# g1mv/density

Hardware: NVIDIA H100
Metric: chameleon_encode_input_GBps (higher is better)
Workload: dtype u32

## Files before the change

### density_b200/csrc/chameleon_encode.cu

```cuda
#include <cstdio>
#include "common.cuh"
#include "encode_internal.cuh"

namespace dns {
namespace cham {

constexpr int TILE_Q = 4096;
__device__ __forceinline__ bool bit_test(const uint32_t* bm, uint32_t i) { return (bm[i >> 5] >> (i & 31)) & 1u; }

constexpr int F6_THREADS = 512, F6_QPT = 8;
constexpr int F6_NW = F6_THREADS / 32, F6_WQ = 32 * F6_QPT;
static_assert(F6_THREADS * F6_QPT == TILE_Q, "tile geometry");
constexpr int F6_MB_SLOTS = 4096, F6_MB_CAP = 4;
constexpr int F6_SEC_SLOTS = 64, F6_SEC_CAP = 16;
#ifdef DNS_PHASE_TIMING
__device__ long long g_f6_ph[8];
#define F6_PH(k) { if (threadIdx.x == 0 && blockIdx.x == 77) { long long tn = clock64(); g_f6_ph[k] += tn - f6_tprev; f6_tprev = tn; } }
#define F6_PH_DECL long long f6_tprev = clock64();
#else
#define F6_PH(k)
#define F6_PH_DECL
#endif
constexpr uint32_t F6_TOUCHED = 1u << 12, F6_DROPPED = 1u << 13;
struct Flag6Smem {
    uint16_t tab[65536];
    uint32_t vbit[2048];
    uint2 rec[TILE_Q];
    union {
        uint16_t mb[F6_MB_SLOTS][F6_MB_CAP];
        uint2 stage[F6_NW][64];
    };
    uint32_t mbcnt[2][F6_MB_SLOTS / 4];
    __align__(16) uint32_t sec[F6_SEC_SLOTS][F6_SEC_CAP];
    uint32_t seccnt[2][F6_SEC_SLOTS];
    uint32_t sigw[2][TILE_Q / 32];
    uint32_t cnt[32];
    uint32_t unres_count;
    uint32_t overflow;
};
static_assert(sizeof(Flag6Smem) <= 227 * 1024, "flag pass shared memory");

__device__ __forceinline__ void f6_append_unres(bool pred, uint32_t qidx_in_run, uint32_t hf, uint32_t* s_count, uint2* __restrict__ unres_run) {
    const uint32_t m = __ballot_sync(0xFFFFFFFFu, pred);
    if (m == 0) return;
    uint32_t base = 0;
    if ((threadIdx.x & 31) == 0) base = atomicAdd(s_count, (uint32_t)__popc(m));
    base = __shfl_sync(0xFFFFFFFFu, base, 0);
    if (pred) {
        const uint32_t idx = base + __popc(m & lanemask_lt());
        if (idx < 65536u) unres_run[idx] = make_uint2(qidx_in_run, hf);
    }
}

static_assert(F6_NW == 16, "one warp per bucket class hash >> 12");
__device__ __forceinline__ void f6_replay_step(Flag6Smem& S, const uint2* stage, uint32_t n, uint32_t buf, uint32_t run_q0,
                                               uint2* __restrict__ unres_run) {
    const uint32_t lane = threadIdx.x & 31;
    const bool valid = lane < n;
    uint2 r = make_uint2(0, 0);
    if (valid) r = stage[lane];
    const uint32_t hh = r.x & 0xFFFFu, ff = r.x >> 16, pos = r.y & 0xFFFu;
    uint32_t cur = 0;
    if (valid) cur = S.tab[hh];
    const uint32_t grp = __match_any_sync(0xFFFFFFFFu, valid ? hh : 0x10000u + lane);
    const uint32_t lower = grp & lanemask_lt();
    const uint32_t fprev = __shfl_sync(0xFFFFFFFFu, ff, lower ? 31 - __clz(lower) : 0);
    bool touched = true, hit;
    if (lower) hit = fprev == ff;
    else {
        if (cur == 0) touched = bit_test(S.vbit, hh);
        hit = touched && cur == ff;
    }
    if (valid && (grp & lanemask_gt()) == 0) {
        S.tab[hh] = (uint16_t)ff;
        if (ff == 0) atomicOr(&S.vbit[hh >> 5], 1u << (hh & 31));
    }
    if (valid && hit) atomicOr(&S.sigw[buf][pos >> 5], 1u << (pos & 31));
    f6_append_unres(valid && !touched, run_q0 + pos, r.x, &S.unres_count, unres_run);
    __syncwarp();
}

__device__ __noinline__ void f6_replay(Flag6Smem& S, uint32_t buf, uint32_t run_q0, uint2* __restrict__ unres_run) {
    const uint32_t lane = threadIdx.x & 31, warp = threadIdx.x >> 5;
    {
        const uint32_t n = S.cnt[warp];
        const uint2* __restrict__ myrec = S.rec + warp * F6_WQ;
        #pragma unroll 1
        for (uint32_t i = lane; i < n; i += 32) {
            const uint2 r = myrec[i];
            S.tab[r.x & 0xFFFFu] = (uint16_t)(r.y >> 16);
        }
    }
    __syncthreads();
    uint2* __restrict__ stage = S.stage[warp];
    uint32_t ns = 0;
    #pragma unroll 1
    for (uint32_t w = 0; w < (uint32_t)F6_NW; ++w) {
        const uint32_t n = S.cnt[w];
        const uint2* __restrict__ rg = S.rec + w * F6_WQ;
        #pragma unroll 1
        for (uint32_t i0 = 0; i0 < n; i0 += 32) {
            const uint32_t i = i0 + lane;
            uint2 r = make_uint2(0, 0);
            if (i < n) r = rg[i];
            const bool mine = i < n && ((r.x & 0xFFFFu) >> 12) == warp;
            const uint32_t m = __ballot_sync(0xFFFFFFFFu, mine);
            if (mine) stage[ns + __popc(m & lanemask_lt())] = r;
            ns += __popc(m);
            if (ns >= 32) {
                __syncwarp();
                f6_replay_step(S, stage, 32, buf, run_q0, unres_run);
                const uint2 rest = stage[32 + lane];
                __syncwarp();
                if (lane < ns - 32) stage[lane] = rest;
                ns -= 32;
                __syncwarp();
            }
        }
    }
    __syncwarp();
    if (ns) f6_replay_step(S, stage, ns, buf, run_q0, unres_run);
}

template <bool GENERIC>
__device__ __forceinline__ void f6_tile(Flag6Smem& S, const uint32_t (&q)[F6_QPT], uint32_t validmask, uint32_t buf, uint32_t run_q0,
                                        uint2* __restrict__ unres_run) {
    const uint32_t tid = threadIdx.x, lane = tid & 31, warp = tid >> 5;
    const uint32_t pos0 = warp * F6_WQ + lane;
    uint32_t h[F6_QPT], f[F6_QPT], old[F6_QPT];
    uint32_t missmask = 0;
    F6_PH_DECL
#pragma unroll
    for (int k = 0; k < F6_MB_SLOTS / 4 / F6_THREADS; ++k) S.mbcnt[buf ^ 1u][tid + k * F6_THREADS] = 0;
    if (tid < F6_SEC_SLOTS) S.seccnt[buf ^ 1u][tid] = 0;
#pragma unroll
    for (int j = 0; j < F6_QPT; ++j) {
        const uint32_t p = hash_prod(q[j]);
        h[j] = prod_hash(p);
        f[j] = prod_fp(p, q[j]);
        old[j] = S.tab[h[j]];
    }
    uint32_t fmin = f[0];
#pragma unroll
    for (int j = 0; j < F6_QPT; ++j) {
        bool miss = old[j] != f[j];
        if (GENERIC) miss = miss && ((validmask >> j) & 1u);
        if (miss) missmask |= 1u << j;
        fmin = min(fmin, f[j]);
    }
    if (fmin == 0) {
#pragma unroll
        for (int j = 0; j < F6_QPT; ++j)
            if (f[j] == 0 && old[j] == 0 && (!GENERIC || ((validmask >> j) & 1u)) && !bit_test(S.vbit, h[j])) missmask |= 1u << j;
    }
    __syncthreads();
    F6_PH(0)
#pragma unroll
    for (int j = 0; j < F6_QPT; ++j)
        if (missmask & (1u << j)) S.tab[h[j]] = (uint16_t)f[j];
    __syncthreads();
    F6_PH(1)
    uint32_t clean[F6_QPT], base = 0;
    uint2* __restrict__ myrec = S.rec + warp * F6_WQ;
#pragma unroll
    for (int j = 0; j < F6_QPT; ++j) {
        bool dirty = (missmask >> j) & 1u;
        if (!dirty) dirty = S.tab[h[j]] != f[j];
        if (GENERIC) dirty = dirty && ((validmask >> j) & 1u);
        const uint32_t db = __ballot_sync(0xFFFFFFFFu, dirty);
        clean[j] = GENERIC ? __ballot_sync(0xFFFFFFFFu, !dirty && ((validmask >> j) & 1u)) : ~db;
        if (dirty) myrec[base + __popc(db & lanemask_lt())] = make_uint2(h[j] | (f[j] << 16), (pos0 + 32 * j) | (old[j] << 16));
        base += __popc(db);
    }
    if (lane == 0) {
#pragma unroll
        for (int j = 0; j < F6_QPT; j += 4)
            *reinterpret_cast<uint4*>(&S.sigw[buf][warp * F6_QPT + j]) = make_uint4(clean[j], clean[j + 1], clean[j + 2], clean[j + 3]);
        S.cnt[warp] = base;
    }
    __syncwarp();
    uint2 r0 = make_uint2(0, 0);
    bool drop0 = false;
    {
        uint32_t carry_x = 0, carry_pos = 0;
        #pragma unroll 1
        for (uint32_t i0 = 0; i0 < base; i0 += 32) {
            const uint32_t i = i0 + lane;
            const bool valid = i < base;
            uint2 r = make_uint2(0xFFFFFFFFu, 0);
            if (valid) {
                r = myrec[i];
                if ((r.y >> 16) != 0 || bit_test(S.vbit, r.x & 0xFFFFu)) r.y |= F6_TOUCHED;
            }
            uint32_t px = __shfl_up_sync(0xFFFFFFFFu, r.x, 1), ppos = __shfl_up_sync(0xFFFFFFFFu, r.y & 0xFFFu, 1);
            if (lane == 0) { px = carry_x; ppos = carry_pos; }
            const bool drop = valid && i != 0 && px == r.x && ppos + 1 == (r.y & 0xFFFu);
            carry_x = __shfl_sync(0xFFFFFFFFu, r.x, 31); carry_pos = __shfl_sync(0xFFFFFFFFu, r.y & 0xFFFu, 31);
            if (i0 == 0) { r0 = r; drop0 = drop; }
            if (drop) {
                const uint32_t pos = r.y & 0xFFFu;
                atomicOr(&S.sigw[buf][pos >> 5], 1u << (pos & 31));
                if (i0) myrec[i].y = r.y | F6_DROPPED;
            } else if (valid) {
                if (i0 && (r.y & F6_TOUCHED)) myrec[i].y = r.y;
                const uint32_t hh = r.x & 0xFFFFu, slot = hh & (F6_MB_SLOTS - 1), sh = (slot & 3u) * 8u;
                const uint32_t k = (atomicAdd(&S.mbcnt[buf][slot >> 2], 1u << sh) >> sh) & 0xFFu;
                if (k < (uint32_t)F6_MB_CAP) S.mb[slot][k] = (uint16_t)(((hh >> 12) << 12) | (warp * F6_WQ + i));
                else {
                    const uint32_t s2 = slot & (F6_SEC_SLOTS - 1);
                    const uint32_t k2 = atomicAdd(&S.seccnt[buf][s2], 1u);
                    if (k2 < (uint32_t)F6_SEC_CAP) S.sec[s2][k2] = (hh << 12) | (warp * F6_WQ + i);
                    else S.overflow = 1;
                }
            }
        }
    }
    __syncthreads();
    F6_PH(2)
#ifdef DNS_PHASE_TIMING
    if (threadIdx.x == 0 && blockIdx.x == 77) { g_f6_ph[6] += S.overflow; uint32_t tot = 0; for (int w = 0; w < F6_NW; ++w) tot += S.cnt[w]; g_f6_ph[7] += tot; }
#endif
    if (S.overflow) {
        f6_replay(S, buf, run_q0, unres_run);
    } else {
        #pragma unroll 1
        for (uint32_t i0 = 0; i0 < base; i0 += 32) {
            const uint32_t i = i0 + lane;
            bool valid = i < base;
            uint2 r = r0;
            if (i0) r = valid ? myrec[i] : make_uint2(0, 0);
            if (i0 ? (r.y & F6_DROPPED) != 0 : drop0) valid = false;
            const uint32_t hh = r.x & 0xFFFFu, ff = r.x >> 16, pos = r.y & 0xFFFu, slot = hh & (F6_MB_SLOTS - 1);
            const uint32_t myidx = warp * F6_WQ + i;
            bool later = false, hit = false, unres = false;
            if (valid) {
                const uint32_t n = (S.mbcnt[buf][slot >> 2] >> ((slot & 3u) * 8u)) & 0xFFu;
                const uint2 e2 = *reinterpret_cast<const uint2*>(&S.mb[slot][0]);
                const uint32_t me = ((hh >> 12) << 12) | myidx;
                int best = -1;
#pragma unroll
                for (int t = 0; t < F6_MB_CAP; ++t) {
                    const uint32_t e = ((t & 2) ? e2.y : e2.x) >> ((t & 1) * 16) & 0xFFFFu;
                    if ((uint32_t)t < n && ((e ^ me) >> 12) == 0) {
                        if (e < me) best = max(best, (int)(e & 0xFFFu));
                        later |= e > me;
                    }
                }
                if (n > (uint32_t)F6_MB_CAP) {
                    const uint32_t s2 = slot & (F6_SEC_SLOTS - 1);
                    const uint32_t n2 = S.seccnt[buf][s2];
                    const uint32_t mine = (hh << 12) | myidx;
                    #pragma unroll 1
                    for (uint32_t t4 = 0; t4 < n2; t4 += 4) {
                        const uint4 e4 = *reinterpret_cast<const uint4*>(&S.sec[s2][t4]);
                        const uint32_t ev[4] = {e4.x, e4.y, e4.z, e4.w};
#pragma unroll
                        for (int t = 0; t < 4; ++t) {
                            const uint32_t e = ev[t];
                            if (t4 + t < n2 && ((e ^ mine) & 0xFFFFF000u) == 0) {
                                if (e < mine) best = max(best, (int)(e & 0xFFFu));
                                later |= e > mine;
                            }
                        }
                    }
                }
                if (best >= 0) hit = (S.rec[best].x >> 16) == ff;
                else if (r.y & F6_TOUCHED) hit = (r.y >> 16) == ff;
                else unres = true;
                if (!later) {
                    S.tab[hh] = (uint16_t)ff;
                    if (ff == 0) atomicOr(&S.vbit[hh >> 5], 1u << (hh & 31));
                }
                if (hit) atomicOr(&S.sigw[buf][pos >> 5], 1u << (pos & 31));
            }
            f6_append_unres(unres, run_q0 + pos, r.x, &S.unres_count, unres_run);
        }
    }
    __syncthreads();
    F6_PH(3)
}

__global__ void __launch_bounds__(F6_THREADS, 1)
cham_flag_pass6(const uint32_t* __restrict__ in, uint64_t nquads, uint32_t tiles_total, uint32_t nruns,
                uint32_t* __restrict__ sigw_g, uint2* __restrict__ unres, uint32_t* __restrict__ unres_count,
                uint32_t* __restrict__ final_tab, const uint8_t* __restrict__ copymap, const Status* __restrict__ gate)
{
    if (gate && !(gate->nonquiet && !gate->converged)) return;
    extern __shared__ __align__(16) unsigned char smem_raw[];
    Flag6Smem& S = *reinterpret_cast<Flag6Smem*>(smem_raw);
    const uint32_t tid = threadIdx.x, lane = tid & 31, warp = tid >> 5;
    const uint32_t run = blockIdx.x;
    const uint64_t t_begin = (uint64_t)run * tiles_total / nruns;
    const uint64_t t_end = (uint64_t)(run + 1) * tiles_total / nruns;
    uint2* __restrict__ unres_run = unres + (size_t)run * 65536;
    const uint32_t pos0 = warp * F6_WQ + lane;
    const uint32_t ntile_run = (uint32_t)(t_end - t_begin);
    const uint64_t q_begin = t_begin * TILE_Q;
    const uint64_t q_end64 = (t_end * TILE_Q < nquads) ? t_end * TILE_Q : nquads;
    const uint32_t run_quads = q_begin < q_end64 ? (uint32_t)(q_end64 - q_begin) : 0u;
    const uint32_t* __restrict__ rin = in + q_begin;
    uint32_t* __restrict__ rsig = sigw_g + t_begin * (TILE_Q / 32);
    const uint8_t* __restrict__ rcm = copymap ? copymap + t_begin * 64 : nullptr;
    {
        const uint4 z = make_uint4(0, 0, 0, 0);
        uint4* t4 = reinterpret_cast<uint4*>(S.tab);
        #pragma unroll 1
        for (uint32_t i = tid; i < 65536 * 2 / 16; i += F6_THREADS) t4[i] = z;
        #pragma unroll 1
        for (uint32_t i = tid; i < 2048; i += F6_THREADS) S.vbit[i] = 0;
        #pragma unroll 1
        for (uint32_t i = tid; i < F6_MB_SLOTS / 4; i += F6_THREADS) { S.mbcnt[0][i] = 0; S.mbcnt[1][i] = 0; }
        if (tid < F6_SEC_SLOTS) { S.seccnt[0][tid] = 0; S.seccnt[1][tid] = 0; }
        if (tid == 0) { S.unres_count = 0; S.overflow = 0; }
    }
    __syncthreads();
    uint32_t nxt[F6_QPT], nxt2[F6_QPT];
#pragma unroll
    for (int j = 0; j < F6_QPT; ++j) {
        nxt[j] = (pos0 + 32 * j < run_quads) ? ld_stream_u32(rin + pos0 + 32 * j) : 0u;
        nxt2[j] = (TILE_Q + pos0 + 32 * j < run_quads) ? ld_stream_u32(rin + TILE_Q + pos0 + 32 * j) : 0u;
    }
    #pragma unroll 1
    for (uint32_t lt = 0; lt < ntile_run; ++lt) {
        uint32_t q[F6_QPT];
        const uint32_t run_q0 = lt * TILE_Q;
        const uint32_t left = run_q0 < run_quads ? run_quads - run_q0 : 0u;
        const uint32_t buf = lt & 1u;
#pragma unroll
        for (int j = 0; j < F6_QPT; ++j) { q[j] = nxt[j]; nxt[j] = nxt2[j]; }
        {
            const uint32_t nleft = left > 2u * TILE_Q ? left - 2u * TILE_Q : 0u;
            const uint32_t* __restrict__ np = rin + run_q0 + 2 * TILE_Q + pos0;
            if (nleft >= (uint32_t)TILE_Q) {
#pragma unroll
                for (int j = 0; j < F6_QPT; ++j) nxt2[j] = ld_stream_u32(np + 32 * j);
            } else {
#pragma unroll
                for (int j = 0; j < F6_QPT; ++j) nxt2[j] = (pos0 + 32 * j < nleft) ? ld_stream_u32(np + 32 * j) : 0u;
            }
        }
        if (left >= (uint32_t)TILE_Q && !rcm) {
            f6_tile<false>(S, q, (1u << F6_QPT) - 1u, buf, run_q0, unres_run);
        } else {
            uint32_t validmask = 0, cp = 0;
            if (rcm) {
#pragma unroll
                for (int b = 0; b < F6_WQ / 64; ++b) cp |= (rcm[lt * 64 + warp * (F6_WQ / 64) + b] ? 1u : 0u) << b;
            }
#pragma unroll
            for (int j = 0; j < F6_QPT; ++j)
                if (pos0 + 32 * j < left && !((cp >> (j >> 1)) & 1u)) validmask |= 1u << j;
            f6_tile<true>(S, q, validmask, buf, run_q0, unres_run);
        }
        if (tid < TILE_Q / 32) rsig[lt * (TILE_Q / 32) + tid] = S.sigw[buf][tid];
        if (tid == 0) S.overflow = 0;
    }
    #pragma unroll 1
    for (uint32_t i = tid; i < 65536; i += F6_THREADS) {
        const uint32_t v = S.tab[i];
        const uint32_t tch = (v != 0 || bit_test(S.vbit, i)) ? 0x10000u : 0u;
        final_tab[(size_t)run * 65536 + i] = v | tch;
    }
    if (tid == 0) unres_count[run] = S.unres_count < 65536u ? S.unres_count : 65536u;
#ifdef DNS_PHASE_TIMING
    if (tid == 0 && run == 77 && ntile_run) { const long long nt = ntile_run;
        printf("f6 run %u tiles %lld cycles/tile: A %lld B %lld C+deposit %lld D+S4 %lld  overflow tiles %lld dirty/tile %lld\n", run, nt, g_f6_ph[0] / nt, g_f6_ph[1] / nt,
               g_f6_ph[2] / nt, g_f6_ph[3] / nt, g_f6_ph[6], g_f6_ph[7] / nt);
        for (int k = 0; k < 8; ++k) g_f6_ph[k] = 0; }
#endif
}

__device__ __forceinline__ bool gate_open(const Status* g) { return !g || (g->nonquiet && !g->converged); }

__global__ void cham_carry_scan(const uint32_t* __restrict__ final_tab, const uint32_t* __restrict__ init, int init_untouched,
                                uint32_t nruns, uint32_t* __restrict__ carry, uint32_t* __restrict__ table_out,
                                const Status* __restrict__ gate = nullptr) {
    if (!gate_open(gate)) return;
    uint32_t hb = blockIdx.x * blockDim.x + threadIdx.x;
    if (hb >= 65536) return;
    uint32_t c = init ? init[hb] : ((hb == 0 && !init_untouched) ? 0x10000u : 0u);
    for (uint32_t r = 0; r < nruns; ++r) {
        if (carry) carry[(size_t)r * 65536 + hb] = c;
        uint32_t v = final_tab[(size_t)r * 65536 + hb];
        if (v & 0x10000u) c = v;
    }
    if (table_out) table_out[hb] = c;
}

__global__ void cham_resolve(const uint2* __restrict__ unres, const uint32_t* __restrict__ unres_count,
                             const uint32_t* __restrict__ carry, uint32_t tiles_total, uint32_t nruns,
                             uint32_t* __restrict__ sigw_g, const Status* __restrict__ gate = nullptr) {
    if (!gate_open(gate)) return;
    const uint32_t run = blockIdx.y;
    const uint32_t n = unres_count[run];
    const uint64_t run_q0 = ((uint64_t)run * tiles_total / nruns) * TILE_Q;
    for (uint32_t i = blockIdx.x * blockDim.x + threadIdx.x; i < n; i += gridDim.x * blockDim.x) {
        uint2 e = unres[(size_t)run * 65536 + i];
        uint32_t c = carry[(size_t)run * 65536 + (e.y & 0xFFFFu)];
        if ((c & 0x10000u) && (c & 0xFFFFu) == (e.y >> 16)) {
            uint64_t gq = run_q0 + e.x;
            atomicOr(&sigw_g[gq >> 5], 1u << (gq & 31));
        }
    }
}

struct ProtSmem {
    uint16_t tab[65536];
    uint32_t vbit[2048];
};

__global__ void __launch_bounds__(1024, 1)
cham_protected_pass(const uint32_t* __restrict__ in, uint64_t nbytes, const Status* __restrict__ status, int only_if_nonquiet,
                    uint32_t* __restrict__ sigw_g, uint8_t* __restrict__ copymap) {
    if (only_if_nonquiet && !(status->nonquiet && !status->converged)) return;
    extern __shared__ __align__(16) unsigned char smem_raw[];
    ProtSmem& S = *reinterpret_cast<ProtSmem*>(smem_raw);
    const uint32_t tid = threadIdx.x, lane = tid & 31;
    {
        uint4 z = make_uint4(0, 0, 0, 0);
        uint4* t4 = reinterpret_cast<uint4*>(S.tab);
        for (uint32_t i = tid; i < 65536 * 2 / 16; i += blockDim.x) t4[i] = z;
        for (uint32_t i = tid; i < 2048; i += blockDim.x) S.vbit[i] = (i == 0) ? 1u : 0u;
    }
    __syncthreads();
    if (tid >= 32) return;

    const uint64_t nquads = nbytes / 4;
    const uint64_t nblocks = (nbytes + 255) / 256;
    Protection ps; ps.init();
    uint32_t n0 = 0, n1 = 0;
    if (nblocks) {
        if (lane < nquads) n0 = in[lane];
        if (32 + lane < nquads) n1 = in[32 + lane];
    }
    for (uint64_t b = 0; b < nblocks; ++b) {
        const uint32_t q0 = n0, q1 = n1;
        {
            uint64_t g = (b + 1) * 64 + lane;
            n0 = (b + 1 < nblocks && g < nquads) ? in[g] : 0u;
            n1 = (b + 1 < nblocks && g + 32 < nquads) ? in[g + 32] : 0u;
        }
        const uint64_t bq0 = b * 64;
        const uint32_t nq = (uint32_t)((nquads - bq0 < 64) ? (nquads - bq0) : 64);
        if (ps.revert_to_copy()) {
            if (lane == 0) { copymap[b] = 1; sigw_g[2 * b] = 0; sigw_g[2 * b + 1] = 0; }
            ps.decay();
            continue;
        }
        uint32_t sig[2];
#pragma unroll
        for (int half = 0; half < 2; ++half) {
            const uint32_t q = half ? q1 : q0;
            const bool valid = half * 32 + lane < nq;
            const uint32_t p = hash_prod(q);
            uint32_t hh = valid ? prod_hash(p) : 0x10000u + lane;
            const uint32_t ff = prod_fp(p, q);
            uint32_t cur = 0; bool touched = false;
            if (valid) { cur = S.tab[hh]; touched = cur != 0 || bit_test(S.vbit, hh); }
            const uint32_t grp = __match_any_sync(0xFFFFFFFFu, hh);
            const uint32_t lower = grp & lanemask_lt();
            const int pl = lower ? 31 - __clz(lower) : 0;
            const uint32_t fprev = __shfl_sync(0xFFFFFFFFu, ff, pl);
            const bool hit = valid && (lower ? (fprev == ff) : (touched && cur == ff));
            const bool is_last = (grp & lanemask_gt()) == 0;
            if (valid && is_last && (lower || !hit)) {
                S.tab[hh] = (uint16_t)ff;
                if (ff == 0) atomicOr(&S.vbit[hh >> 5], 1u << (hh & 31));
            }
            sig[half] = __ballot_sync(0xFFFFFFFFu, hit);
            __syncwarp();
        }
        if (lane == 0) { copymap[b] = 0; sigw_g[2 * b] = sig[0]; sigw_g[2 * b + 1] = sig[1]; }
        const uint32_t hits = __popc(sig[0]) + __popc(sig[1]);
        const uint32_t tailb = (b == nblocks - 1) ? (uint32_t)(nbytes & 3) : 0u;
        const uint32_t out_sz = 8 + 4 * nq - 2 * hits + tailb;
        ps.update(out_sz >= 256);
    }
}

constexpr int PSEG = 256;

__device__ __forceinline__ uint32_t prot_pack(const Protection& ps) { return ps.copy_penalty | (ps.copy_penalty_start << 8) | (ps.previous_incompressible << 16); }
__device__ __forceinline__ void prot_walk(Protection& ps, const uint8_t* __restrict__ inc, uint64_t b0, uint64_t b1, uint8_t* __restrict__ cm) {
    for (uint64_t b = b0; b < b1; ++b) {
        if (ps.revert_to_copy()) { cm[b] = 1; ps.decay(); }
        else { cm[b] = 0; ps.update(__ldcg(&inc[b]) != 0); }
    }
}
constexpr int PROT_ROUNDS = 48, PROT_FAST_ROUNDS = 4;
constexpr int PI_THREADS = 1024;

constexpr uint32_t PC_NS = 10, PC_NP = 10, PC_NC = 2 * PC_NS * PC_NP, PC_ESC = 0xFFFFu, PC_GROUP = 128;
__host__ __device__ __forceinline__ size_t prot_table_elems(uint64_t nseg) {
    const uint64_t ngrp = (nseg + PC_GROUP - 1) / PC_GROUP;
    return (size_t)(2 * (ngrp + 2) + nseg * PC_NC + ngrp * PC_NC + 64);
}
__device__ __forceinline__ void pc_decode(uint32_t c, Protection& ps) {
    ps.copy_penalty = c % PC_NP; ps.copy_penalty_start = (c / PC_NP) % PC_NS + 1u; ps.previous_incompressible = c / (PC_NP * PC_NS);
}
__device__ __forceinline__ uint32_t pc_encode(const Protection& ps) {
    if (ps.copy_penalty >= PC_NP || ps.copy_penalty_start < 1u || ps.copy_penalty_start > PC_NS) return PC_ESC;
    return (ps.previous_incompressible * PC_NS + (ps.copy_penalty_start - 1u)) * PC_NP + ps.copy_penalty;
}

__device__ __forceinline__ void grid_barrier(unsigned int* counter, unsigned int nctas, unsigned int& epoch) {
    __syncthreads();
    if (threadIdx.x == 0) {
        __threadfence();
        atomicAdd(counter, 1u);
        const unsigned int target = (epoch + 1) * nctas;
        while (atomicAdd(counter, 0u) < target) { __nanosleep(64); }
        __threadfence();
    }
    ++epoch;
    __syncthreads();
}

__device__ unsigned long long g_prot_dbg[16][2];

__global__ void __launch_bounds__(PI_THREADS)
prot_iterate(const uint32_t* __restrict__ sigw_g, uint64_t nbytes, uint64_t nblocks, uint32_t nseg, Status* __restrict__ st, int it,
             uint8_t* __restrict__ inc, uint8_t* __restrict__ cm_old, uint8_t* __restrict__ cm_new,
             uint32_t* __restrict__ in_state, uint32_t* __restrict__ out_state, uint16_t* __restrict__ ptab) {
    if (!gate_open(st)) return;
    __shared__ uint32_t s_state[1024], s_in[1024];
    __shared__ uint8_t s_inc[PSEG], s_cm[PSEG];
    __shared__ uint32_t s_cur, s_redo;
    const uint32_t tid = threadIdx.x;
    const uint64_t gtid = (uint64_t)blockIdx.x * PI_THREADS + tid, gsz = (uint64_t)gridDim.x * PI_THREADS;
    unsigned int epoch = 0;
    unsigned int* bar = &st->barrier[it & 7];

    if (sigw_g)
        for (uint64_t b = gtid; b < nblocks; b += gsz)
            if (!(it && cm_old[b])) inc[b] = (nbytes - b * 256 >= 256) && (__popc(sigw_g[2 * b]) + __popc(sigw_g[2 * b + 1]) <= 4);
    if (gtid == 0) { st->relax_changed[0] = 0; st->relax_changed[1] = 0; st->iter_changed = 0; st->pad2[0] = 0; }
    if (gtid < 16 && it == 0) { g_prot_dbg[gtid][0] = ~0ull; g_prot_dbg[gtid][1] = 0; }
    grid_barrier(bar, gridDim.x, epoch);

    bool settled = false;
    int round = 0;
    for (int phase = 0; phase < 2 && !settled; ++phase) {
    const int limit = (phase == 0 && ptab) ? PROT_FAST_ROUNDS : PROT_ROUNDS;
    for (; round < limit; ++round) {
        for (uint64_t s = gtid; s < nseg; s += gsz) {
            const uint32_t new_in = (s && round) ? __ldcg(&out_state[s - 1]) : (1u << 8);
            if (round > 0 && new_in == in_state[s]) continue;
            Protection ps;
            ps.copy_penalty = new_in & 0xFFu; ps.copy_penalty_start = (new_in >> 8) & 0xFFu; ps.previous_incompressible = (new_in >> 16) & 1u;
            ps.counter = s * PSEG;
            const uint64_t b1 = ((s + 1) * PSEG < nblocks) ? (s + 1) * PSEG : nblocks;
            prot_walk(ps, inc, s * PSEG, b1, cm_new);
            in_state[s] = new_in;
            out_state[s] = prot_pack(ps);
            if (round > 0) st->relax_changed[round & 1] = 1;
            else if (prot_pack(ps) != (1u << 8)) atomicAdd(&st->pad2[0], 1u);
        }
        grid_barrier(bar, gridDim.x, epoch);
        if (round == 0 && phase == 0 && ptab) {
            const unsigned int bad = *((volatile unsigned int*)&st->pad2[0]);
            if (bad == 0) { settled = true; break; }
            if (bad > 8u) { round = 1; break; }
        }
        if (round > 0) {
            const bool changed = *((volatile unsigned int*)&st->relax_changed[round & 1]) != 0;
            if (!changed) { settled = true; break; }
        }
        if (gtid == 0) st->relax_changed[(round + 1) & 1] = 0;
        grid_barrier(bar, gridDim.x, epoch);
    }
    if (phase == 0 && !settled && ptab) {
        const uint32_t ngrp = (nseg + PC_GROUP - 1) / PC_GROUP;
        uint32_t* gin = reinterpret_cast<uint32_t*>(ptab);
        uint16_t* T = ptab + 2 * (ngrp + 2);
        uint16_t* GT = T + (size_t)nseg * PC_NC;
        for (uint64_t idx = gtid; idx < (uint64_t)nseg * PC_NC; idx += gsz) {
            const uint64_t s = idx / PC_NC;
            Protection ps; pc_decode((uint32_t)(idx % PC_NC), ps);
            ps.counter = s * PSEG;
            const uint64_t b1 = ((s + 1) * PSEG < nblocks) ? (s + 1) * PSEG : nblocks;
            uint64_t b = s * PSEG;
            for (; b + 16 <= b1; b += 16) {
                const uint4 v = __ldcg(reinterpret_cast<const uint4*>(inc + b));
                const uint32_t w[4] = {v.x, v.y, v.z, v.w};
#pragma unroll
                for (int k = 0; k < 16; ++k) {
                    if (ps.revert_to_copy()) ps.decay();
                    else ps.update(((w[k >> 2] >> ((k & 3) * 8)) & 0xFFu) != 0);
                }
            }
            for (; b < b1; ++b) {
                if (ps.revert_to_copy()) ps.decay();
                else ps.update(__ldcg(&inc[b]) != 0);
            }
            T[idx] = (uint16_t)pc_encode(ps);
        }
        grid_barrier(bar, gridDim.x, epoch);
        for (uint64_t idx = gtid; idx < (uint64_t)ngrp * PC_NC; idx += gsz) {
            const uint32_t g = (uint32_t)(idx / PC_NC);
            uint32_t x = (uint32_t)(idx % PC_NC);
            const uint32_t s1 = ((g + 1) * PC_GROUP < nseg) ? (g + 1) * PC_GROUP : nseg;
            for (uint32_t s = g * PC_GROUP; s < s1 && x != PC_ESC; ++s) x = __ldcg(&T[(size_t)s * PC_NC + x]);
            GT[idx] = (uint16_t)x;
        }
        grid_barrier(bar, gridDim.x, epoch);
        if (gtid == 0) {
            uint32_t x = 0;
            for (uint32_t g = 0; g < ngrp; ++g) { gin[g] = x; if (x != PC_ESC) x = __ldcg(&GT[(size_t)g * PC_NC + x]); }
            gin[ngrp] = x;
        }
        grid_barrier(bar, gridDim.x, epoch);
        if (__ldcg(&gin[ngrp]) != PC_ESC) {
            for (uint64_t g = gtid; g < ngrp; g += gsz) {
                uint32_t x = __ldcg(&gin[g]);
                const uint32_t s1 = ((g + 1) * PC_GROUP < nseg) ? (uint32_t)((g + 1) * PC_GROUP) : nseg;
                for (uint32_t s = (uint32_t)g * PC_GROUP; s < s1; ++s) { in_state[s] = x; x = __ldcg(&T[(size_t)s * PC_NC + x]); }
            }
            grid_barrier(bar, gridDim.x, epoch);
            for (uint64_t s = gtid; s < nseg; s += gsz) {
                Protection ps; pc_decode(__ldcg(&in_state[s]), ps);
                ps.counter = s * PSEG;
                const uint64_t b1 = ((s + 1) * PSEG < nblocks) ? (s + 1) * PSEG : nblocks;
                prot_walk(ps, inc, s * PSEG, b1, cm_new);
            }
            grid_barrier(bar, gridDim.x, epoch);
            settled = true;
        }
    }

    }

    if (!settled) {
        if (blockIdx.x == 0) {
            if (tid == 0) s_cur = 1u << 8;
            for (uint32_t s0 = 0; s0 < nseg; s0 += 1024) {
                __syncthreads();
                for (uint32_t i = tid; i < 1024 && s0 + i < nseg; i += PI_THREADS) { s_state[i] = __ldcg(&out_state[s0 + i]); s_in[i] = __ldcg(&in_state[s0 + i]); }
                __syncthreads();
                const uint32_t cnt = (nseg - s0 < 1024u) ? (nseg - s0) : 1024u;
                uint32_t i = 0;
                while (i < cnt) {
                    if (tid == 0) {
                        uint32_t cur = s_cur;
                        while (i < cnt && cur == s_in[i]) { cur = s_state[i]; ++i; }
                        s_cur = cur;
                        s_redo = (i < cnt) ? i : 0xFFFFFFFFu;
                    }
                    __syncthreads();
                    const uint32_t r = s_redo;
                    if (r == 0xFFFFFFFFu) break;
                    const uint64_t b0 = (uint64_t)(s0 + r) * PSEG;
                    const uint32_t nb = (uint32_t)((nblocks - b0 < (uint64_t)PSEG) ? (nblocks - b0) : PSEG);
                    if (tid < nb) s_inc[tid] = __ldcg(&inc[b0 + tid]);
                    __syncthreads();
                    if (tid == 0) {
                        Protection ps; const uint32_t c = s_cur;
                        ps.copy_penalty = c & 0xFFu; ps.copy_penalty_start = (c >> 8) & 0xFFu; ps.previous_incompressible = (c >> 16) & 1u; ps.counter = b0;
// ... 938 lines not shown
```

Baseline: 480.9.

## Micro-optimize flag6 tile hashing, dedup scan, mailbox lookup and tile loop indexing

Several instruction-level changes land in the flag6 tile kernel. The hash and fingerprint are now computed with __umulhi instead of the helper functions. The record-store branch is restructured, and the shuffle-based neighbour comparison in the dedup scan is replaced by re-reading the previous record from shared memory. The 4-way mailbox search loop becomes branchless min arithmetic, and the tile loop uses pointer increments and a precomputed full-tile count. The aim is to cut ALU and shuffle work per quad, at the risk of subtle semantic differences, for example in the umulhi-based hash and in the min-based best/later computation.

```diff
diff --git a/density_b200/csrc/chameleon_encode.cu b/density_b200/csrc/chameleon_encode.cu
--- a/density_b200/csrc/chameleon_encode.cu
+++ b/density_b200/csrc/chameleon_encode.cu
@@ -136,8 +136,8 @@
 #pragma unroll
     for (int j = 0; j < F6_QPT; ++j) {
         const uint32_t p = hash_prod(q[j]);
-        h[j] = prod_hash(p);
-        f[j] = prod_fp(p, q[j]);
+        h[j] = __umulhi(p, 0x10000u);
+        f[j] = __umulhi(q[j], 2u) + (p - h[j] * 0x10000u);
         old[j] = S.tab[h[j]];
     }
     uint32_t fmin = f[0];
@@ -162,14 +162,19 @@
     F6_PH(1)
     uint32_t clean[F6_QPT], base = 0;
     uint2* __restrict__ myrec = S.rec + warp * F6_WQ;
+    const uint32_t ltmask = lanemask_lt();
 #pragma unroll
     for (int j = 0; j < F6_QPT; ++j) {
-        bool dirty = (missmask >> j) & 1u;
-        if (!dirty) dirty = S.tab[h[j]] != f[j];
+        const bool miss = (missmask >> j) & 1u;
+        uint32_t now = f[j];
+        if (!miss) now = S.tab[h[j]];
+        bool dirty = miss || now != f[j];
         if (GENERIC) dirty = dirty && ((validmask >> j) & 1u);
         const uint32_t db = __ballot_sync(0xFFFFFFFFu, dirty);
         clean[j] = GENERIC ? __ballot_sync(0xFFFFFFFFu, !dirty && ((validmask >> j) & 1u)) : ~db;
-        if (dirty) myrec[base + __popc(db & lanemask_lt())] = make_uint2(h[j] | (f[j] << 16), (pos0 + 32 * j) | (old[j] << 16));
+        const uint2 rv = make_uint2(f[j] * 0x10000u + h[j], old[j] * 0x10000u + (pos0 + 32 * j));
+        const uint32_t k = base + __popc(db & ltmask);
+        if (dirty) myrec[k] = rv;
         base += __popc(db);
     }
     if (lane == 0) {
@@ -182,20 +187,19 @@
     uint2 r0 = make_uint2(0, 0);
     bool drop0 = false;
     {
-        uint32_t carry_x = 0, carry_pos = 0;
         #pragma unroll 1
         for (uint32_t i0 = 0; i0 < base; i0 += 32) {
             const uint32_t i = i0 + lane;
             const bool valid = i < base;
-            uint2 r = make_uint2(0xFFFFFFFFu, 0);
-            if (valid) {
-                r = myrec[i];
-                if ((r.y >> 16) != 0 || bit_test(S.vbit, r.x & 0xFFFFu)) r.y |= F6_TOUCHED;
-            }
-            uint32_t px = __shfl_up_sync(0xFFFFFFFFu, r.x, 1), ppos = __shfl_up_sync(0xFFFFFFFFu, r.y & 0xFFFu, 1);
-            if (lane == 0) { px = carry_x; ppos = carry_pos; }
-            const bool drop = valid && i != 0 && px == r.x && ppos + 1 == (r.y & 0xFFFu);
-            carry_x = __shfl_sync(0xFFFFFFFFu, r.x, 31); carry_pos = __shfl_sync(0xFFFFFFFFu, r.y & 0xFFFu, 31);
+            uint2 r = make_uint2(0xFFFFFFFFu, 0), pr = r;
+            __syncwarp();
+            if (valid) r = myrec[i];
+            if (valid && i != 0) pr = myrec[i - 1];
+            __syncwarp();
+            uint32_t tch = r.y >> 16;
+            if (valid && tch == 0) tch = S.vbit[(r.x & 0xFFFFu) >> 5] & (1u << (r.x & 31u));
+            if (valid && tch != 0) r.y |= F6_TOUCHED;
+            const bool drop = valid && i != 0 && pr.x == r.x && (((pr.y + 1u) ^ r.y) & 0xFFFu) == 0;
             if (i0 == 0) { r0 = r; drop0 = drop; }
             if (drop) {
                 const uint32_t pos = r.y & 0xFFFu;
@@ -236,16 +240,13 @@
             if (valid) {
                 const uint32_t n = (S.mbcnt[buf][slot >> 2] >> ((slot & 3u) * 8u)) & 0xFFu;
                 const uint2 e2 = *reinterpret_cast<const uint2*>(&S.mb[slot][0]);
-                const uint32_t me = ((hh >> 12) << 12) | myidx;
-                int best = -1;
-#pragma unroll
-                for (int t = 0; t < F6_MB_CAP; ++t) {
-                    const uint32_t e = ((t & 2) ? e2.y : e2.x) >> ((t & 1) * 16) & 0xFFFFu;
-                    if ((uint32_t)t < n && ((e ^ me) >> 12) == 0) {
-                        if (e < me) best = max(best, (int)(e & 0xFFFu));
-                        later |= e > me;
-                    }
-                }
+                const uint32_t me = (hh & 0xF000u) | myidx;
+                const uint32_t ea = e2.x & 0xFFFFu, eb = n > 1 ? e2.x >> 16 : me, ec = n > 2 ? e2.y & 0xFFFFu : me,
+                               ed = n > 3 ? e2.y >> 16 : me;
+                const uint32_t dmin = min(min(me - ea - 1u, me - eb - 1u), min(me - ec - 1u, me - ed - 1u));
+                const uint32_t umin = min(min(ea - me - 1u, eb - me - 1u), min(ec - me - 1u, ed - me - 1u));
+                int best = dmin < myidx ? (int)(myidx - 1u - dmin) : -1;
+                later = umin < 0xFFFu - myidx;
                 if (n > (uint32_t)F6_MB_CAP) {
                     const uint32_t s2 = slot & (F6_SEC_SLOTS - 1);
                     const uint32_t n2 = S.seccnt[buf][s2];
@@ -320,28 +321,28 @@
         nxt[j] = (pos0 + 32 * j < run_quads) ? ld_stream_u32(rin + pos0 + 32 * j) : 0u;
         nxt2[j] = (TILE_Q + pos0 + 32 * j < run_quads) ? ld_stream_u32(rin + TILE_Q + pos0 + 32 * j) : 0u;
     }
+    const uint32_t nfull = run_quads / TILE_Q;
+    const uint32_t* __restrict__ np = rin + 2 * TILE_Q + pos0;
+    uint32_t* __restrict__ sp = rsig + tid;
     #pragma unroll 1
-    for (uint32_t lt = 0; lt < ntile_run; ++lt) {
+    for (uint32_t lt = 0; lt < ntile_run; ++lt, np += TILE_Q, sp += TILE_Q / 32) {
         uint32_t q[F6_QPT];
         const uint32_t run_q0 = lt * TILE_Q;
-        const uint32_t left = run_q0 < run_quads ? run_quads - run_q0 : 0u;
         const uint32_t buf = lt & 1u;
 #pragma unroll
         for (int j = 0; j < F6_QPT; ++j) { q[j] = nxt[j]; nxt[j] = nxt2[j]; }
-        {
-            const uint32_t nleft = left > 2u * TILE_Q ? left - 2u * TILE_Q : 0u;
-            const uint32_t* __restrict__ np = rin + run_q0 + 2 * TILE_Q + pos0;
-            if (nleft >= (uint32_t)TILE_Q) {
-#pragma unroll
-                for (int j = 0; j < F6_QPT; ++j) nxt2[j] = ld_stream_u32(np + 32 * j);
-            } else {
-#pragma unroll
-                for (int j = 0; j < F6_QPT; ++j) nxt2[j] = (pos0 + 32 * j < nleft) ? ld_stream_u32(np + 32 * j) : 0u;
-            }
-        }
-        if (left >= (uint32_t)TILE_Q && !rcm) {
+        if (lt + 2 < nfull) {
+#pragma unroll
+            for (int j = 0; j < F6_QPT; ++j) nxt2[j] = ld_stream_u32(np + 32 * j);
+        } else {
+            const uint32_t nleft = run_q0 + 2u * TILE_Q < run_quads ? run_quads - run_q0 - 2u * TILE_Q : 0u;
+#pragma unroll
+            for (int j = 0; j < F6_QPT; ++j) nxt2[j] = (pos0 + 32 * j < nleft) ? ld_stream_u32(np + 32 * j) : 0u;
+        }
+        if (lt < nfull && !rcm) {
             f6_tile<false>(S, q, (1u << F6_QPT) - 1u, buf, run_q0, unres_run);
         } else {
+            const uint32_t left = run_q0 < run_quads ? run_quads - run_q0 : 0u;
             uint32_t validmask = 0, cp = 0;
             if (rcm) {
 #pragma unroll
@@ -352,7 +353,7 @@
                 if (pos0 + 32 * j < left && !((cp >> (j >> 1)) & 1u)) validmask |= 1u << j;
             f6_tile<true>(S, q, validmask, buf, run_q0, unres_run);
         }
-        if (tid < TILE_Q / 32) rsig[lt * (TILE_Q / 32) + tid] = S.sigw[buf][tid];
+        if (tid < TILE_Q / 32) *sp = S.sigw[buf][tid];
         if (tid == 0) S.overflow = 0;
     }
     #pragma unroll 1
```

Result: faster. 495.8 (median of 6 runs) (+3.1%).
